# gwenzhang/GGA

Hardware: AMD Instinct MI355X
Metric: kitti_frames_per_sec_gga_train_step (higher is better)
Workload: dtype f32 tensors; products on 2 x f16 operand planes (block-scaled), f32 accumulate - measured no less accurate than fp32 kernels: per convolution 0.7 x (dense) / 0.7-1.2 x (sparse) the RMS error of an fp32 FMA chain vs float64, whole-step losses over 8 seeds <= 2.5e-5 from float64 (fp32 CPU step: <= 1.6

## Files before the change

gga_amd/csrc/dense_conv.h:

```cpp
#pragma once
#include "gga_common.h"
#include "conv_planes.h"

#define DC_TW 32
#define DC_HW (DC_TW + 2)
#define DC_CK 16
#define DC_WS_MAX_CIN 4096
#define DC_ROWB 48

struct DcBnBwd {
    const float* y;
    const float* gamma;
    const float* beta;
    const float* mean;
    const float* invstd;
    int ystride;
};

#define DC_MAX_SLICES 16
struct DcSlices {
    int n;
    const uint16_t* w[DC_MAX_SLICES];
    float* y[DC_MAX_SLICES];
    double* stats[DC_MAX_SLICES];
};

int dc_tile_rows(int B, int H, int W, int cout, int planes);
int64_t dc_ws_grid(int64_t n_tiles);
bool dc_ws_enabled(int planes);
int dc_launch_ws(const float* x, const void* split_weight, int B, int H, int W, int cin, int cout, float* y, int ystride, int prow,
                 int pcol, double* stats, const uint32_t* amax_x, const uint32_t* amax_weight, DcBnBwd bn, const DcSlices* slices,
                 hipStream_t stream);
```

gga_amd/csrc/dense_conv.hip:

```cpp
#include <stdlib.h>

#include "dense_conv.h"
#include <type_traits>
#include <hip/hip_fp16.h>

#define X9_SIX 1
#ifndef DC_PIPE_ON
#define DC_PIPE_ON 1
#endif
#ifndef DC_PIPE4_ON
#define DC_PIPE4_ON 1
#endif
#define DC_P4_MAX_TILES 256

#define DC_MAX_ENTRIES 16
struct DcLevels {
    int n;
    int start[DC_MAX_ENTRIES + 1];
    int H[DC_MAX_ENTRIES], W[DC_MAX_ENTRIES];
    const float* x[DC_MAX_ENTRIES];
    float* y[DC_MAX_ENTRIES];
    const uint16_t* w[DC_MAX_ENTRIES];
    const uint32_t* amax_x[DC_MAX_ENTRIES];
    const float* bias[DC_MAX_ENTRIES];
// ... 508 lines not shown
                sl.w[e] = (const uint16_t*)split_weight[e]; sl.y[e] = y[e]; sl.stats[e] = stats ? stats[e] : nullptr;
            }
            DcBnBwd nobn;
            nobn.y = nullptr; nobn.gamma = nobn.beta = nobn.mean = nobn.invstd = nullptr; nobn.ystride = 0;
            const int H = transposed ? widths[0] : heights[0], W = transposed ? heights[0] : widths[0];
            return dc_launch_ws(x[0], split_weight[0], B, H, W, cin, cout, y[0], (int)y_pixel_stride, transposed ? 1 : widths[0],
                                transposed ? widths[0] : 1, stats ? stats[0] : nullptr, amax_x[0], amax_weight, nobn, &sl, stream);
        }
    }
    DcLevels lv;
    lv.n = n_entries;
    int64_t total = 0;
    for (int e = 0; e < n_entries; ++e) {
        GGA_REQUIRE(x[e] && y[e] && split_weight[e] && heights[e] >= 1 && widths[e] >= 1 &&
                        (int64_t)heights[e] * widths[e] * cin < 2147483647ll && (planes == 3 || amax_x[e]),
                    "gga_dense_conv3x3_levels: bad entry %d", e);
        lv.start[e] = (int)total;
        lv.H[e] = heights[e]; lv.W[e] = widths[e];
        lv.x[e] = x[e]; lv.y[e] = y[e]; lv.w[e] = (const uint16_t*)split_weight[e];
        lv.amax_x[e] = planes == 2 ? amax_x[e] : nullptr;
        lv.bias[e] = bias ? bias[e] : nullptr;
        lv.stats[e] = stats ? stats[e] : nullptr;
        const int th = transposed ? widths[e] : heights[e], tw = transposed ? heights[e] : widths[e];
        total += (int64_t)B * ((tw + DC_TW - 1) / DC_TW) * ((th + tile_rows - 1) / tile_rows);
        GGA_REQUIRE(total < 2147483647ll, "gga_dense_conv3x3_levels: too many tiles");
    }
    lv.start[n_entries] = (int)total;
    lv.transposed = transposed ? 1 : 0;
    for (int e = n_entries + 1; e <= DC_MAX_ENTRIES; ++e) lv.start[e] = (int)total;
    DcBnBwd bn;
    bn.y = nullptr; bn.gamma = bn.beta = bn.mean = bn.invstd = nullptr; bn.ystride = 0;
    const dim3 grid((unsigned)total), block(tile_rows * 32);
#define DC_LV(NT_, TR_, NP_) hipLaunchKernelGGL((dense_conv3x3_x9_kernel<NT_, TR_, NP_, 2>), grid, block, 0, stream, x[0], (const uint16_t*)split_weight[0], B, heights[0], widths[0], cin, cout, 1, 1, y[0], (int)y_pixel_stride, widths[0], 1, (double*)nullptr, planes == 2 ? amax_x[0] : nullptr, amax_weight, bn, lv)
    if (planes == 3) { if (cout == 64) DC_LV(2, 8, 3); else if (tile_rows == 16) DC_LV(4, 16, 3); else DC_LV(4, 8, 3); }
    else {
        if (cout == 64) DC_LV(2, 8, 2);
        else if (tile_rows == 16) DC_LV(4, 16, 2);
        else if (DC_PIPE4_ON && total <= DC_P4_MAX_TILES)
            hipLaunchKernelGGL((dense_conv3x3_x9_kernel<4, 8, 2, 2, 1>), grid, block, 0, stream, x[0], (const uint16_t*)split_weight[0], B, heights[0], widths[0], cin, cout, 1, 1, y[0], (int)y_pixel_stride, widths[0], 1, (double*)nullptr, planes == 2 ? amax_x[0] : nullptr, amax_weight, bn, lv);
        else DC_LV(4, 8, 2);
    }
#undef DC_LV
    GGA_CHECK_LAUNCH("dense_conv3x3_x9_kernel (levels)");
    return GGA_OK;
}

extern "C" int gga_dense_conv3x3_stats(const float* x, const void* split_weight, int B, int H, int W, int cin, int cout,
                                       float* y, double* stats, void* stream) {
    return gga_dense_conv3x3_slice(x, split_weight, B, H, W, cin, cout, y, cout, 0, stats, stream);
}

extern "C" int gga_dense_conv3x3(const float* x, const void* split_weight, int B, int H, int W, int cin, int cout,
                                 float* y, void* stream) {
    return gga_dense_conv3x3_slice(x, split_weight, B, H, W, cin, cout, y, cout, 0, nullptr, stream);
}

#define DW_XPL (2 * 34 * 64)
#define DW_XROW (NP * DW_XPL)
#define DW_GPL (2 * 32 * 64)
#define DW_GROW (NP * DW_GPL)

template <int NP>
__global__ __launch_bounds__(256, 2) void dense_wgrad3x3_x9_kernel(const float* __restrict__ X, const float* __restrict__ G,
                                                                  int B, int H, int W, int cin, int cout, int strips,
                                                                  int prow, int pcol, float* __restrict__ partials,
                                                                  const uint32_t* __restrict__ amax_x,
                                                                  const uint32_t* __restrict__ amax_g, int xblk, int gblk) {
    float xscale = 1.0f, gscale = 1.0f;
    if (NP == 2) {
        const int ncb = cout >> 6;
        xscale = h2_scale(h2_scale_exp(amax_x[xblk ? (int)(blockIdx.y / ncb) : 0]));
        gscale = h2_scale(h2_scale_exp(amax_g[gblk ? (int)(blockIdx.y % ncb) : 0]));
    }
    __shared__ __attribute__((aligned(16))) unsigned char Xs[4 * DW_XROW];
    __shared__ __attribute__((aligned(16))) unsigned char Gs[2 * DW_GROW];
    const int tid = threadIdx.x, lane = tid & 63, wave = tid >> 6;
    const int ti = wave >> 1, tj = wave & 1;
    const int ncb_o = cout >> 6;
    const int ci0 = (blockIdx.y / ncb_o) * 64, co0 = (blockIdx.y % ncb_o) * 64;
    const int64_t total_rows = (int64_t)B * strips * H;
    const int64_t r0 = total_rows * blockIdx.x / gridDim.x, r1 = total_rows * (blockIdx.x + 1) / gridDim.x;
    int x0 = 0, ye = 0;
    const float* Xb = X;
    const float* Gb = G;

    mf_v16 acc[9];
#pragma unroll
    for (int t = 0; t < 9; ++t)
#pragma unroll
        for (int i = 0; i < 16; ++i) acc[t][i] = 0.0f;

    float4 rg0, rg1, rx0, rx1, rx2;
    uint32_t gof0 = 0, gof1 = 0, xof0 = 0, xof1 = 0, xof2 = 0;
    float gs0 = 0.f, gs1 = 0.f, xs0 = 0.f, xs1 = 0.f, xs2 = 0.f;
#define DW_COLG(OF, SC_, E) { const int f = tid + 256 * (E); const int px = f >> 4, q = f & 15; const bool ok = x0 + px < W;      \
        OF = (uint32_t)(((x0 + (ok ? px : 0)) * pcol * cout + 4 * q) * 4); SC_ = ok ? gscale : 0.0f; }
#define DW_COLX(OF, SC_, E) { const int f = tid + 256 * (E); const int px = f >> 4, q = f & 15; const int ix = x0 - 1 + px;       \
        const bool ok = f < 544 && (unsigned)ix < (unsigned)W;                                                        \
        OF = (uint32_t)(((ok ? ix : x0) * pcol * cin + 4 * q) * 4); SC_ = ok ? xscale : 0.0f; }
#define DW_LOAD_G(Y) { const char* rp_ = reinterpret_cast<const char*>(Gb + (int64_t)(Y) * prow * cout);              \
        rg0 = *reinterpret_cast<const float4*>(rp_ + gof0); rg1 = *reinterpret_cast<const float4*>(rp_ + gof1); }
#define DW_LOAD_X(Y) { const int yy = (Y); const int yc_ = yy < 0 ? 0 : (yy < H ? yy : H - 1);                        \
        const char* rp_ = reinterpret_cast<const char*>(Xb + (int64_t)yc_ * prow * cin);                              \
        rx0 = *reinterpret_cast<const float4*>(rp_ + xof0); rx1 = *reinterpret_cast<const float4*>(rp_ + xof1);       \
        rx2 = *reinterpret_cast<const float4*>(rp_ + xof2); }
#define DW_SPLIT_STORE(V, BASE, PL, NPX, F, SC) { const int f = (F); const int px = f >> 4, q = f & 15;               \
        unsigned char* dst = (BASE) + (q >> 3) * ((NPX) * 64) + px * 64 + (q & 7) * 8;                                \
        if (NP == 3) {                                                                                                \
            uint32_t lo1, lo2, lo3, hi1, hi2, hi3;                                                                    \
            x9_split2(V.x * (SC), V.y * (SC), lo1, lo2, lo3); x9_split2(V.z * (SC), V.w * (SC), hi1, hi2, hi3);      \
            *reinterpret_cast<uint2*>(dst) = make_uint2(lo1, hi1);                                                    \
            *reinterpret_cast<uint2*>(dst + (PL)) = make_uint2(lo2, hi2);                                             \
            *reinterpret_cast<uint2*>(dst + (NP - 1) * (PL)) = make_uint2(lo3, hi3);                                  \
        } else {                                                                                                      \
            uint32_t lo1, lo2, hi1, hi2;                                                                              \
            h2_split2s(V.x, V.y, (SC), lo1, lo2); h2_split2s(V.z, V.w, (SC), hi1, hi2);                         \
            *reinterpret_cast<uint2*>(dst) = make_uint2(lo1, hi1);                                                    \
            *reinterpret_cast<uint2*>(dst + (PL)) = make_uint2(lo2, hi2);                                             \
        } }
#define DW_STORE_G(Y) { unsigned char* base = Gs + ((Y) & 1) * DW_GROW;                                               \
        DW_SPLIT_STORE(rg0, base, DW_GPL, 32, tid, gs0) DW_SPLIT_STORE(rg1, base, DW_GPL, 32, tid + 256, gs1) }
#define DW_STORE_X(Y) { unsigned char* base = Xs + (((Y) + 4) & 3) * DW_XROW;                                         \
        const bool rowok_ = (unsigned)(Y) < (unsigned)H;                             \
        const float s0_ = rowok_ ? xs0 : 0.0f, s1_ = rowok_ ? xs1 : 0.0f, s2_ = rowok_ ? xs2 : 0.0f;                 \
        DW_SPLIT_STORE(rx0, base, DW_XPL, 34, tid, s0_) DW_SPLIT_STORE(rx1, base, DW_XPL, 34, tid + 256, s1_)         \
        if (tid + 512 < 544) DW_SPLIT_STORE(rx2, base, DW_XPL, 34, tid + 512, s2_) }

    const int grp = lane >> 4, li = lane & 15;
    const int froff = ((8 * (grp >> 1) + (li >> 2)) * 64) + (16 * (grp & 1) + 4 * (li & 3)) * 2;
    union Frag { mf_v8bf v; dw_v4s h[2]; };
#define DW_FRAG(F, PTR) { F.h[0] = __builtin_amdgcn_ds_read_tr16_b64_v4i16((__attribute__((address_space(3))) dw_v4s*)((PTR) + froff));          \
                          F.h[1] = __builtin_amdgcn_ds_read_tr16_b64_v4i16((__attribute__((address_space(3))) dw_v4s*)((PTR) + froff + 4 * 64)); }

    int64_t idx = r0;
    while (idx < r1) {
    const int col = (int)(idx / H);
    const int ys = (int)(idx - (int64_t)col * H);
    {
        const int b = col / strips, strip = col - b * strips;
        x0 = strip * 32;
        Xb = X + (int64_t)b * H * W * cin + ci0;
        Gb = G + (int64_t)b * H * W * cout + co0;
        DW_COLG(gof0, gs0, 0) DW_COLG(gof1, gs1, 1)
        DW_COLX(xof0, xs0, 0) DW_COLX(xof1, xs1, 1) DW_COLX(xof2, xs2, 2)
    }
    ye = (int)(r1 - idx < (int64_t)(H - ys) ? ys + (r1 - idx) : H);
    idx += ye - ys;
    DW_LOAD_X(ys - 1); DW_STORE_X(ys - 1);
    DW_LOAD_X(ys);     DW_STORE_X(ys);
    DW_LOAD_X(ys + 1); DW_STORE_X(ys + 1);
    DW_LOAD_G(ys);     DW_STORE_G(ys);
    __syncthreads();
    for (int y = ys; y < ye; ++y) {
        const bool more = y + 1 < ye;
        if (more) { DW_LOAD_G(y + 1); DW_LOAD_X(y + 2); }
        const unsigned char* gbase = Gs + (y & 1) * DW_GROW + tj * (32 * 64);
#pragma unroll
        for (int s = 0; s < 2; ++s) {
            Frag g0, g1, g2;
            DW_FRAG(g0, gbase + (16 * s) * 64);
            DW_FRAG(g1, gbase + DW_GPL + (16 * s) * 64);
            if (NP == 3) { DW_FRAG(g2, gbase + (NP - 1) * DW_GPL + (16 * s) * 64); } else g2 = g1;
            if (NP == 2) {
#pragma unroll
                for (int ky = 0; ky < 3; ++ky) {
                    Frag b0[3], b1[3];
#pragma unroll
                    for (int kx = 0; kx < 3; ++kx) {
                        const unsigned char* xb = Xs + ((y + ky - 1 + 4) & 3) * DW_XROW + ti * (34 * 64) + (16 * s + kx) * 64;
                        DW_FRAG(b0[kx], xb);
                        DW_FRAG(b1[kx], xb + DW_XPL);
                    }
#define DW_MI(A_, G_, T_) acc[T_] = __builtin_amdgcn_mfma_f32_32x32x16_f16(__builtin_bit_cast(mf_v8h, A_.v), __builtin_bit_cast(mf_v8h, G_.v), acc[T_], 0, 0, 0);
                    DW_MI(b0[0], g1, 3 * ky) DW_MI(b0[1], g1, 3 * ky + 1) DW_MI(b0[2], g1, 3 * ky + 2)
                    DW_MI(b1[0], g0, 3 * ky) DW_MI(b1[1], g0, 3 * ky + 1) DW_MI(b1[2], g0, 3 * ky + 2)
                    DW_MI(b0[0], g0, 3 * ky) DW_MI(b0[1], g0, 3 * ky + 1) DW_MI(b0[2], g0, 3 * ky + 2)
#undef DW_MI
                }
                continue;
            }
#pragma unroll
            for (int tap = 0; tap < 9; ++tap) {
                const int ky = tap / 3, kx = tap - ky * 3;
                const unsigned char* xbase = Xs + ((y + ky - 1 + 4) & 3) * DW_XROW + ti * (34 * 64) + (16 * s + kx) * 64;
                Frag a0, a1, a2;
                DW_FRAG(a0, xbase);
                DW_FRAG(a1, xbase + DW_XPL);
                if (NP == 2) {
#define DW_MH(A_, G_) acc[tap] = __builtin_amdgcn_mfma_f32_32x32x16_f16(__builtin_bit_cast(mf_v8h, A_.v), __builtin_bit_cast(mf_v8h, G_.v), acc[tap], 0, 0, 0);
                    DW_MH(a0, g1) DW_MH(a1, g0) DW_MH(a0, g0)
#undef DW_MH
                    continue;
                }
                DW_FRAG(a2, xbase + (NP - 1) * DW_XPL);
                acc[tap] = __builtin_amdgcn_mfma_f32_32x32x16_bf16(a0.v, g2.v, acc[tap], 0, 0, 0);
                acc[tap] = __builtin_amdgcn_mfma_f32_32x32x16_bf16(a1.v, g1.v, acc[tap], 0, 0, 0);
                acc[tap] = __builtin_amdgcn_mfma_f32_32x32x16_bf16(a2.v, g0.v, acc[tap], 0, 0, 0);
                acc[tap] = __builtin_amdgcn_mfma_f32_32x32x16_bf16(a0.v, g1.v, acc[tap], 0, 0, 0);
                acc[tap] = __builtin_amdgcn_mfma_f32_32x32x16_bf16(a1.v, g0.v, acc[tap], 0, 0, 0);
                acc[tap] = __builtin_amdgcn_mfma_f32_32x32x16_bf16(a0.v, g0.v, acc[tap], 0, 0, 0);
            }
        }
        if (more) { DW_STORE_G(y + 1); DW_STORE_X(y + 2); }
        __syncthreads();
    }
    }
#undef DW_LOAD_G
#undef DW_COLG
#undef DW_COLX
#undef DW_LOAD_X
#undef DW_SPLIT_STORE
#undef DW_STORE_G
#undef DW_STORE_X
#undef DW_FRAG
    float* out = partials + ((int64_t)blockIdx.y * gridDim.x + blockIdx.x) * (9 * 64 * 64);
    const int r = lane & 31, h = lane >> 5;
#pragma unroll
    for (int tap = 0; tap < 9; ++tap)
#pragma unroll
        for (int v = 0; v < 16; ++v) {
            const int ci = ti * 32 + (v >> 2) * 8 + h * 4 + (v & 3);
            out[(tap * 64 + ci) * 64 + tj * 32 + r] = acc[tap][v];
        }
}

__global__ __launch_bounds__(256) void dense_wgrad_reduce_kernel(const float* __restrict__ partials, int nblk, int cin, int cout,
                                                                int64_t s_co, int64_t s_ci, int64_t s_ky, int64_t s_kx,
                                                                const uint32_t* __restrict__ amax_x,
                                                                const uint32_t* __restrict__ amax_g, int xblk, int gblk,
                                                                float* __restrict__ dW) {
    const int i = blockIdx.x * 256 + threadIdx.x;
    if (i >= 9 * 64 * 64) return;
    const int ncb_o = cout >> 6;
    const int ci0 = (blockIdx.y / ncb_o) * 64, co0 = (blockIdx.y % ncb_o) * 64;
    const float* p = partials + (int64_t)blockIdx.y * nblk * (9 * 64 * 64) + i;
    double s = 0.0;
#pragma unroll 8
    for (int k = 0; k < nblk; ++k) s += (double)p[(int64_t)k * (9 * 64 * 64)];
    const int co = i & 63, ci = (i >> 6) & 63, tap = i >> 12;
    const int ky = tap / 3, kx = tap - ky * 3;
    if (amax_x)
        s = s * (double)h2_descale(h2_scale_exp(amax_x[xblk ? ci0 >> 6 : 0])) * (double)h2_descale(h2_scale_exp(amax_g[gblk ? co0 >> 6 : 0]));
    dW[(co0 + co) * s_co + (ci0 + ci) * s_ci + ky * s_ky + kx * s_kx] = (float)s;
}

static int dense_wgrad_blocks(int B, int H, int W, int cin, int cout) {
    const int64_t total_rows = (int64_t)B * ((W + 31) / 32) * H;
    int64_t n = 512 / ((int64_t)(cin >> 6) * (cout >> 6));
    if (n < 1) n = 1;
    if (n > total_rows) n = total_rows;
    return (int)n;
}

extern "C" size_t gga_dense_wgrad3x3_workspace_bytes(int B, int H, int W, int cin, int cout) {
    if (B < 1 || H < 1 || W < 1 || cin < 64 || cout < 64 || (cin & 63) || (cout & 63)) return 0;
    const int n0 = dense_wgrad_blocks(B, H, W, cin, cout), n1 = dense_wgrad_blocks(B, W, H, cin, cout);
    return (size_t)(n0 > n1 ? n0 : n1) * (cin >> 6) * (cout >> 6) * 9 * 64 * 64 * sizeof(float);
}

extern "C" int gga_dense_wgrad3x3(const float* x, const float* grad_y, int B, int H, int W, int cin, int cout,
                                  float* grad_weight, int64_t stride_co, int64_t stride_ci, int64_t stride_ky,
                                  int64_t stride_kx, int transposed, void* workspace, size_t workspace_bytes,
                                  void* stream_) {
    return gga_dense_wgrad3x3_planes(x, grad_y, B, H, W, cin, cout, grad_weight, stride_co, stride_ci, stride_ky, stride_kx,
                                     transposed, 3, nullptr, nullptr, workspace, workspace_bytes, stream_);
}

extern "C" int gga_dense_wgrad3x3_planes(const float* x, const float* grad_y, int B, int H, int W, int cin, int cout,
                                         float* grad_weight, int64_t stride_co, int64_t stride_ci, int64_t stride_ky,
                                         int64_t stride_kx, int transposed, int planes, const uint32_t* amax_x,
                                         const uint32_t* amax_grad_y, void* workspace, size_t workspace_bytes, void* stream_) {
    return gga_dense_wgrad3x3_block_amax(x, grad_y, B, H, W, cin, cout, grad_weight, stride_co, stride_ci, stride_ky, stride_kx,
                                         transposed, planes, amax_x, 0, amax_grad_y, 0, workspace, workspace_bytes, stream_);
}

extern "C" int gga_dense_wgrad3x3_block_amax(const float* x, const float* grad_y, int B, int H, int W, int cin, int cout,
                                             float* grad_weight, int64_t stride_co, int64_t stride_ci, int64_t stride_ky,
                                             int64_t stride_kx, int transposed, int planes, const uint32_t* amax_x,
                                             int amax_x_per_block, const uint32_t* amax_grad_y, int amax_grad_y_per_block,
                                             void* workspace, size_t workspace_bytes, void* stream_) {
    hipStream_t stream = (hipStream_t)stream_;
    const int xblk = amax_x_per_block ? 1 : 0, gblk = amax_grad_y_per_block ? 1 : 0;
    GGA_REQUIRE(x && grad_y && grad_weight && workspace, "gga_dense_wgrad3x3: null pointer argument");
    GGA_REQUIRE(planes == 3 || (planes == 2 && amax_x && amax_grad_y),
                "gga_dense_wgrad3x3: planes must be 3 (bf16) or 2 (fp16, with the operands' absmax bits)");
    GGA_REQUIRE(B >= 1 && H >= 1 && W >= 1 && cin >= 64 && cout >= 64 && (cin & 63) == 0 && (cout & 63) == 0,
                "gga_dense_wgrad3x3: cin and cout must be multiples of 64 (got %d -> %d)", cin, cout);
    GGA_REQUIRE((int64_t)H * W * (cin > cout ? cin : cout) * 4 < ((int64_t)1 << 31),
                "gga_dense_wgrad3x3: one image of an operand must stay below 2 GiB (32-bit piece offsets; got %d x %d x %d channels)", H, W,
                cin > cout ? cin : cout);
    if (workspace_bytes < gga_dense_wgrad3x3_workspace_bytes(B, H, W, cin, cout)) {
        gga_set_error("gga_dense_wgrad3x3: workspace too small");
        return GGA_ERR_WORKSPACE;
    }
    const int prow = transposed ? 1 : W, pcol = transposed ? W : 1;
    if (transposed) { const int t = H; H = W; W = t; const int64_t ts = stride_ky; stride_ky = stride_kx; stride_kx = ts; }
    const int strips = (W + 31) / 32;
    const int nblk = dense_wgrad_blocks(B, H, W, cin, cout), ncb = (cin >> 6) * (cout >> 6);
    hipEvent_t* tev = gga_timing_acquire(GGA_TIME_DENSE_WGRAD, GGA_TIMING_CONV_KEY(cin, cout, (int64_t)H * W));
    GGA_TIME_START(tev, stream);
    if (planes == 3)
        hipLaunchKernelGGL(dense_wgrad3x3_x9_kernel<3>, dim3(nblk, ncb), dim3(256), 0, stream, x, grad_y, B, H, W, cin, cout, strips,
                           prow, pcol, (float*)workspace, amax_x, amax_grad_y, xblk, gblk);
    else
        hipLaunchKernelGGL(dense_wgrad3x3_x9_kernel<2>, dim3(nblk, ncb), dim3(256), 0, stream, x, grad_y, B, H, W, cin, cout, strips,
                           prow, pcol, (float*)workspace, amax_x, amax_grad_y, xblk, gblk);
    GGA_CHECK_LAUNCH("dense_wgrad3x3_x9_kernel");
    hipLaunchKernelGGL(dense_wgrad_reduce_kernel, dim3((9 * 64 * 64 + 255) / 256, ncb), dim3(256), 0, stream,
                       (const float*)workspace, nblk, cin, cout, stride_co, stride_ci, stride_ky, stride_kx,
                       planes == 2 ? amax_x : nullptr, amax_grad_y, xblk, gblk, grad_weight);
    GGA_CHECK_LAUNCH("dense_wgrad_reduce_kernel");
    GGA_TIME_STOP(tev, stream);
    return GGA_OK;
}
```

Measured before the change: 519.8.

## Add warp-specialized producer/consumer kernel for two-plane dense weight gradient

After: 524.7, median of 6. Within noise of the previous version (+0.9%).

```diff
diff --git a/gga_amd/csrc/dense_conv.h b/gga_amd/csrc/dense_conv.h
--- a/gga_amd/csrc/dense_conv.h
+++ b/gga_amd/csrc/dense_conv.h
@@ -31,3 +31,7 @@
 int dc_launch_ws(const float* x, const void* split_weight, int B, int H, int W, int cin, int cout, float* y, int ystride, int prow,
                  int pcol, double* stats, const uint32_t* amax_x, const uint32_t* amax_weight, DcBnBwd bn, const DcSlices* slices,
                  hipStream_t stream);
+bool dw_ws_enabled(int planes);
+void dw_ws_launch(dim3 grid, hipStream_t stream, const float* x, const float* grad_y, int B, int H, int W, int cin, int cout,
+                  int strips, int prow, int pcol, float* partials, const uint32_t* amax_x, const uint32_t* amax_grad_y, int xblk,
+                  int gblk);
diff --git a/gga_amd/csrc/dense_conv.hip b/gga_amd/csrc/dense_conv.hip
--- a/gga_amd/csrc/dense_conv.hip
+++ b/gga_amd/csrc/dense_conv.hip
@@ -834,6 +834,9 @@
     if (planes == 3)
         hipLaunchKernelGGL(dense_wgrad3x3_x9_kernel<3>, dim3(nblk, ncb), dim3(256), 0, stream, x, grad_y, B, H, W, cin, cout, strips,
                            prow, pcol, (float*)workspace, amax_x, amax_grad_y, xblk, gblk);
+    else if (dw_ws_enabled(planes))
+        dw_ws_launch(dim3(nblk, ncb), stream, x, grad_y, B, H, W, cin, cout, strips, prow, pcol, (float*)workspace, amax_x,
+                     amax_grad_y, xblk, gblk);
     else
         hipLaunchKernelGGL(dense_wgrad3x3_x9_kernel<2>, dim3(nblk, ncb), dim3(256), 0, stream, x, grad_y, B, H, W, cin, cout, strips,
                            prow, pcol, (float*)workspace, amax_x, amax_grad_y, xblk, gblk);
diff --git a/gga_amd/csrc/dense_wgrad_ws.hip b/gga_amd/csrc/dense_wgrad_ws.hip
--- /dev/null
+++ b/gga_amd/csrc/dense_wgrad_ws.hip
@@ -0,0 +1,13 @@
+#include "dense_wgrad_ws_kernels.h"
+
+bool dw_ws_enabled(int planes) {
+    const char* e = getenv("GGA_DW_WS");
+    return planes == 2 && !(e && atoi(e) == 0);
+}
+
+void dw_ws_launch(dim3 grid, hipStream_t stream, const float* x, const float* grad_y, int B, int H, int W, int cin, int cout,
+                  int strips, int prow, int pcol, float* partials, const uint32_t* amax_x, const uint32_t* amax_grad_y, int xblk,
+                  int gblk) {
+    hipLaunchKernelGGL(dense_wgrad3x3_ws_kernel<2>, grid, dim3(512), 0, stream, x, grad_y, B, H, W, cin, cout, strips, prow, pcol,
+                       partials, amax_x, amax_grad_y, xblk, gblk);
+}
diff --git a/gga_amd/csrc/dense_wgrad_ws_kernels.h b/gga_amd/csrc/dense_wgrad_ws_kernels.h
--- /dev/null
+++ b/gga_amd/csrc/dense_wgrad_ws_kernels.h
@@ -0,0 +1,206 @@
+#pragma once
+#include <stdlib.h>
+
+#include <type_traits>
+
+#include "dense_conv.h"
+
+#define DWS_XPL (2 * 34 * 64)
+#define DWS_XROW (2 * DWS_XPL)
+#define DWS_GPL (2 * 32 * 64)
+#define DWS_GROW (2 * DWS_GPL)
+#define DWS_XR 12
+#define DWS_GR 4
+
+struct DwsSet {
+    float4 g[2];
+    float gs[2];
+    float4 x[3][3];
+    float xs[3][3];
+    int nx;
+    int seq;
+    int gslot;
+};
+
+template <int NP>
+__global__ __launch_bounds__(512, 2) void dense_wgrad3x3_ws_kernel(const float* __restrict__ X, const float* __restrict__ G,
+                                                                    int B, int H, int W, int cin, int cout, int strips,
+                                                                    int prow, int pcol, float* __restrict__ partials,
+                                                                    const uint32_t* __restrict__ amax_x,
+                                                                    const uint32_t* __restrict__ amax_g, int xblk, int gblk) {
+    static_assert(NP == 2, "the producer / consumer weight gradient runs the two-plane arithmetic only");
+    const int ncb_o = cout >> 6;
+    const float xscale = h2_scale(h2_scale_exp(amax_x[xblk ? (int)(blockIdx.y / ncb_o) : 0]));
+    const float gscale = h2_scale(h2_scale_exp(amax_g[gblk ? (int)(blockIdx.y % ncb_o) : 0]));
+    __shared__ __attribute__((aligned(16))) unsigned char Xs[DWS_XR * DWS_XROW];
+    __shared__ __attribute__((aligned(16))) unsigned char Gs[DWS_GR * DWS_GROW];
+    const int tid = threadIdx.x, lane = tid & 63;
+    const int wave = __builtin_amdgcn_readfirstlane(tid >> 6);
+    const int ci0 = (blockIdx.y / ncb_o) * 64, co0 = (blockIdx.y % ncb_o) * 64;
+    const int64_t total_rows = (int64_t)B * strips * H;
+    const int64_t r0 = total_rows * blockIdx.x / gridDim.x, r1 = total_rows * (blockIdx.x + 1) / gridDim.x;
+    const int n = (int)(r1 - r0);
+    const int y_first = (int)(r0 % H);
+
+    if (wave >= 4) {
+        const int ptid = tid - 256;
+        int ly = y_first, lnb = 0;
+        int64_t lcol = r0 / H;
+        const float* Xb = X;
+        const float* Gb = G;
+        uint32_t gof[2] = {0, 0}, xof[3] = {0, 0, 0};
+        float gsc[2] = {0.f, 0.f}, xsc[3] = {0.f, 0.f, 0.f};
+        bool first = true;
+        auto fetch = [&](DwsSet& S, int j) {
+            const bool start = first || ly == 0;
+            first = false;
+            if (start) {
+                const int b = (int)(lcol / strips), strip = (int)(lcol - (int64_t)b * strips);
+                const int x0 = strip * 32;
+                Xb = X + (int64_t)b * H * W * cin + ci0;
+                Gb = G + (int64_t)b * H * W * cout + co0;
+#pragma unroll
+                for (int e = 0; e < 2; ++e) {
+                    const int f = ptid + 256 * e, px = f >> 4, q = f & 15;
+                    const bool ok = x0 + px < W;
+                    gof[e] = (uint32_t)(((x0 + (ok ? px : 0)) * pcol * cout + 4 * q) * 4);
+                    gsc[e] = ok ? gscale : 0.0f;
+                }
+#pragma unroll
+                for (int e = 0; e < 3; ++e) {
+                    const int f = ptid + 256 * e, px = f >> 4, q = f & 15, ix = x0 - 1 + px;
+                    const bool ok = f < 544 && (unsigned)ix < (unsigned)W;
+                    xof[e] = (uint32_t)(((ok ? ix : x0) * pcol * cin + 4 * q) * 4);
+                    xsc[e] = ok ? xscale : 0.0f;
+                }
+            }
+            {
+                const char* rp = reinterpret_cast<const char*>(Gb + (int64_t)ly * prow * cout);
+#pragma unroll
+                for (int e = 0; e < 2; ++e) { S.g[e] = *reinterpret_cast<const float4*>(rp + gof[e]); S.gs[e] = gsc[e]; }
+            }
+#pragma unroll
+            for (int i = 0; i < 3; ++i) {
+                if (i > 0 && !start) break;
+                const int yy = start ? ly - 1 + i : ly + 1;
+                const bool rowok = (unsigned)yy < (unsigned)H;
+                const int yc = yy < 0 ? 0 : (yy < H ? yy : H - 1);
+                const char* rp = reinterpret_cast<const char*>(Xb + (int64_t)yc * prow * cin);
+#pragma unroll
+                for (int e = 0; e < 3; ++e) {
+                    S.x[i][e] = *reinterpret_cast<const float4*>(rp + xof[e]);
+                    S.xs[i][e] = rowok ? xsc[e] : 0.0f;
+                }
+            }
+            S.nx = start ? 3 : 1;
+            S.seq = start ? lnb : lnb + 2;
+            S.gslot = j % DWS_GR;
+            if (++ly == H) { ly = 0; ++lcol; }
+            lnb += ly == 0 ? 3 : 1;
+        };
+        auto split_store = [&](const float4& v, unsigned char* base, int pl, int npx, int f, float sc) {
+            const int px = f >> 4, q = f & 15;
+            unsigned char* dst = base + (q >> 3) * (npx * 64) + px * 64 + (q & 7) * 8;
+            uint32_t lo1, lo2, hi1, hi2;
+            h2_split2s(v.x, v.y, sc, lo1, lo2); h2_split2s(v.z, v.w, sc, hi1, hi2);
+            *reinterpret_cast<uint2*>(dst) = make_uint2(lo1, hi1);
+            *reinterpret_cast<uint2*>(dst + pl) = make_uint2(lo2, hi2);
+        };
+        auto store = [&](const DwsSet& S) {
+            unsigned char* gb = Gs + S.gslot * DWS_GROW;
+            split_store(S.g[0], gb, DWS_GPL, 32, ptid, S.gs[0]);
+            split_store(S.g[1], gb, DWS_GPL, 32, ptid + 256, S.gs[1]);
+#pragma unroll
+            for (int i = 0; i < 3; ++i) {
+                if (i >= S.nx) break;
+                unsigned char* xb = Xs + ((S.seq + i) % DWS_XR) * DWS_XROW;
+                split_store(S.x[i][0], xb, DWS_XPL, 34, ptid, S.xs[i][0]);
+                split_store(S.x[i][1], xb, DWS_XPL, 34, ptid + 256, S.xs[i][1]);
+                if (ptid + 512 < 544) split_store(S.x[i][2], xb, DWS_XPL, 34, ptid + 512, S.xs[i][2]);
+            }
+        };
+        DwsSet s0, s1;
+        fetch(s0, 0); store(s0);
+        if (n > 1) { fetch(s1, 1); store(s1); }
+        if (n > 2) fetch(s0, 2);
+        if (n > 3) fetch(s1, 3);
+        __syncthreads();
+        for (int k = 0; k < n; k += 2) {
+            if (k + 2 < n) store(s0);
+            if (k + 4 < n) fetch(s0, k + 4);
+            __syncthreads();
+            if (k + 1 >= n) break;
+            if (k + 3 < n) store(s1);
+            if (k + 5 < n) fetch(s1, k + 5);
+            __syncthreads();
+        }
+        return;
+    }
+
+    const int ti = wave >> 1;
+    const int grp = lane >> 4, li = lane & 15;
+    int froff = ((8 * (grp >> 1) + (li >> 2)) * 64) + (16 * (grp & 1) + 4 * (li & 3)) * 2;
+    union Frag { mf_v8bf v; dw_v4s h[2]; };
+    auto consume = [&](auto parity) {
+        constexpr int P = decltype(parity)::value;
+        constexpr int AKY = P ? 2 : 0;
+        constexpr int BKX[3] = {P, P ? 2 : 0, P ? 2 : 1}, BTJ[3] = {P, P ? 0 : 1, P ? 1 : 0};
+        mf_v16 acc[9];
+#pragma unroll
+        for (int t = 0; t < 9; ++t)
+#pragma unroll
+            for (int i = 0; i < 16; ++i) acc[t][i] = 0.0f;
+#define DWS_FRAG(F, PTR) { F.h[0] = __builtin_amdgcn_ds_read_tr16_b64_v4i16((__attribute__((address_space(3))) dw_v4s*)((PTR) + froff));          \
+                           F.h[1] = __builtin_amdgcn_ds_read_tr16_b64_v4i16((__attribute__((address_space(3))) dw_v4s*)((PTR) + froff + 4 * 64)); }
+#define DWS_READ_X(FX, SEQ, S_, KX0, NKX) {                                                                           \
+            const unsigned char* xb_ = Xs + ((SEQ) % DWS_XR) * DWS_XROW + ti * (34 * 64) + (16 * (S_) + (KX0)) * 64;   \
+            _Pragma("unroll") for (int j = 0; j < (NKX); ++j) { DWS_FRAG(FX[j], xb_ + j * 64) DWS_FRAG(FX[(NKX) + j], xb_ + j * 64 + DWS_XPL) } }
+#define DWS_READ_G(FG, GSLOT, S_) {                                                                                   \
+            const unsigned char* gb_ = Gs + (GSLOT) * DWS_GROW + (16 * (S_)) * 64;                                     \
+            _Pragma("unroll") for (int t = 0; t < 2; ++t) { DWS_FRAG(FG[2 * t], gb_ + t * (32 * 64)) DWS_FRAG(FG[2 * t + 1], gb_ + t * (32 * 64) + DWS_GPL) } }
+#define DWS_MI(A_, G_, T_) acc[T_] = __builtin_amdgcn_mfma_f32_32x32x16_f16(__builtin_bit_cast(mf_v8h, A_.v), __builtin_bit_cast(mf_v8h, G_.v), acc[T_], 0, 0, 0);
+#define DWS_MMA_A(FX, FG) {                                                                                           \
+            _Pragma("unroll") for (int t = 0; t < 6; ++t) DWS_MI(FX[t >> 1], FG[2 * (t & 1) + 1], t)                    \
+            _Pragma("unroll") for (int t = 0; t < 6; ++t) DWS_MI(FX[3 + (t >> 1)], FG[2 * (t & 1)], t)                  \
+            _Pragma("unroll") for (int t = 0; t < 6; ++t) DWS_MI(FX[t >> 1], FG[2 * (t & 1)], t) }
+#define DWS_MMA_B(FX, FG) {                                                                                           \
+            _Pragma("unroll") for (int t = 0; t < 3; ++t) DWS_MI(FX[BKX[t] - P], FG[2 * BTJ[t] + 1], 6 + t)            \
+            _Pragma("unroll") for (int t = 0; t < 3; ++t) DWS_MI(FX[2 + BKX[t] - P], FG[2 * BTJ[t]], 6 + t)            \
+            _Pragma("unroll") for (int t = 0; t < 3; ++t) DWS_MI(FX[BKX[t] - P], FG[2 * BTJ[t]], 6 + t) }
+        Frag xa[6], xb[4], fg[2][4];
+        int nb = 0, cy = y_first;
+        __syncthreads();
+        DWS_READ_G(fg[0], 0, 0)
+        DWS_READ_X(xa, nb + AKY, 0, 0, 3)
+        for (int k = 0; k < n; ++k) {
+            const int nb1 = nb + (cy + 1 == H ? 3 : 1);
+            const int gs = k % DWS_GR, gs1 = (k + 1) % DWS_GR;
+            DWS_READ_X(xb, nb + 1, 0, P, 2)                              DWS_MMA_A(xa, fg[0])
+            DWS_READ_G(fg[1], gs, 1) DWS_READ_X(xa, nb + AKY, 1, 0, 3)    DWS_MMA_B(xb, fg[0])
+            DWS_READ_X(xb, nb + 1, 1, P, 2)                              DWS_MMA_A(xa, fg[1])
+            DWS_READ_G(fg[0], gs1, 0) DWS_READ_X(xa, nb1 + AKY, 0, 0, 3)  DWS_MMA_B(xb, fg[1])
+            asm volatile("s_barrier" : "+v"(froff));
+            nb = nb1;
+            cy = cy + 1 == H ? 0 : cy + 1;
+        }
+#undef DWS_MMA_A
+#undef DWS_MMA_B
+#undef DWS_MI
+#undef DWS_READ_G
+#undef DWS_READ_X
+#undef DWS_FRAG
+        float* out = partials + ((int64_t)blockIdx.y * gridDim.x + blockIdx.x) * (9 * 64 * 64);
+        const int r = lane & 31, h = lane >> 5;
+#pragma unroll
+        for (int t = 0; t < 9; ++t) {
+            const int tap = t < 6 ? 3 * AKY + (t >> 1) : 3 + BKX[t - 6], tj = t < 6 ? (t & 1) : BTJ[t - 6];
+#pragma unroll
+            for (int v = 0; v < 16; ++v) {
+                const int ci = ti * 32 + (v >> 2) * 8 + h * 4 + (v & 3);
+                out[(tap * 64 + ci) * 64 + tj * 32 + r] = acc[t][v];
+            }
+        }
+    };
+    if (wave & 1) consume(std::integral_constant<int, 1>());
+    else consume(std::integral_constant<int, 0>());
+}
```
